# Maaz77/Head-Pose-Estimation-Model

Measured on AMD Instinct MI355X. Metric: images/sec (train+infer) on 96×96 feature maps; yaw/pitch/roll MAE vs ref, higher is better.
Workload: dtype fp32; 1 GPU; Model-96 create_model(num_filters=360, dropout=0, l2=0.1) training, legacy Adam lr 2.8e-4, 96x96 feature maps (configs[3] per GPU: 512 images per rank); global_batch=512, per_gpu_batch=512, positions_per_image=9216, channels=96, parallelism=dp1

## Files before the change

head-pose-estimation-model_amd/csrc/hpe_mlp2.hip:

```cpp
#include <hip/hip_runtime.h>
#include <stdint.h>
#include <stdlib.h>

#include "hpe_common.h"
#include "hpe_dev.h"

#ifdef MLP2_BIG
#define MLP2_NS mlp2_big
#else
#define MLP2_NS mlp2_small
#endif
#define MLP2_BIG_ROWS (1 << 15)
namespace MLP2_NS {

#define MLP2_MAXW 12
#ifndef MLP2_BAR1_SKIP
#define MLP2_BAR1_SKIP 1
#endif
#ifndef MLP2_W88
#define MLP2_W88 2
#endif
#define MLP2_XS 100
#define MLP2_XF (32 * MLP2_XS)
#define MLP2_LAB 128
#define MLP2_RED 32
#define MLP2_FS 104
#define MLP2_TS 40
#define MLP2_A1W (15 * 68 + 64)
#define MLP2_PRE_HALVES (3 * 32 * MLP2_FS + 2 * 3 * 96 * MLP2_TS)

struct E2 {
  int act, drop;
  uint32_t thr;
  float keep;
};

struct TileImg {
  int img0, rem0, P;
  __device__ __forceinline__ int of(int r) const {
    const int t = rem0 + r;
    return img0 + (P >= 32 ? (t >= P ? 1 : 0) : (P == 1 ? t : t / P));
  }
  __device__ __forceinline__ void advance(int dq, int dr) {
    img0 += dq;
    rem0 += dr;
    if (rem0 >= P) { rem0 -= P; ++img0; }
  }
};

__device__ __forceinline__ float e_fwd(const E2& e, uint64_t seed, int64_t img, int ch, float z) {
  float a = act_f(e.act, z);
  if (e.drop >= 0) a = drop_hash(seed, e.drop, (uint64_t)img, ch) >= e.thr ? a / e.keep : 0.f;
  return a;
}

__device__ __forceinline__ float e_bwd(const E2& e, uint64_t seed, int64_t img, int ch, float g, float val) {
  if (e.drop >= 0) {
    if (drop_hash(seed, e.drop, (uint64_t)img, ch) < e.thr) return 0.f;
    g = g / e.keep;
    val = val * e.keep;
  }
  return e.act == ACT_LINEAR ? g : g * act_grad(e.act, val, 0.f);
}
// ... 22 lines not shown
  }
  const int lr = min(lane & 31, last);
  const int limg = ti.of(lr);
  const int lpos = (int)(row0 + lr - (int64_t)limg * P);
  const int lsrc = args.idx ? args.idx[limg] : limg;
  __builtin_amdgcn_s_waitcnt(0x0F70);
  if (labels && wave == 0) {
#pragma unroll
    for (int pc = 0; pc < 2; ++pc) {
      const int slot = pc * 64 + lane;
      const int r = min(slot >> 2, last), j = min(slot & 3, 2);
      const int64_t src = __shfl(lsrc, r, 64);
      glds4(args.ytrue + src * 3 + j, lds_addr(lab + pc * 64));
    }
  }
  for (int r = wave; r < 32; r += NCB) {
    const int rr = min(r, last);
    const int64_t srow = (int64_t)__builtin_amdgcn_readlane(lsrc, rr) * P +
                         __builtin_amdgcn_readlane(lpos, rr);
    if (lane < q) glds16(args.x + srow * Cin + 4 * lane, lds_addr(xs + r * XS));
  }
}

typedef _Float16 h4 __attribute__((ext_vector_type(4)));

__device__ __forceinline__ void split_d4(f32x4 v, h4& ch, h4& cl, h4& h) {
  const f32x4 s = v * SPLIT_C;
  ch = __builtin_convertvector(s, h4);
  cl = __builtin_convertvector(s - __builtin_convertvector(ch, f32x4), h4);
  h = __builtin_convertvector(v, h4);
}
__device__ __forceinline__ constexpr int a1_row(int g) { return 68 * (g ^ ((g >> 1) & 4)); }
template <int KH>
__device__ __forceinline__ void presplit_tile(const float* xs, _Float16* xf, _Float16* xt, int tid, int NT) {
  for (int i = tid; i < 32 * 24; i += NT) {
    const int r = i / 24, rem = i - r * 24, h = rem >= 12 ? 1 : 0, m0 = 4 * (rem - 12 * h);
    const f32x4 v = m0 < KH ? *(const f32x4*)(xs + r * MLP2_XS + KH * h + m0) : f32x4{0.f, 0.f, 0.f, 0.f};
    h4 ch, cl, hh;
    split_d4(v, ch, cl, hh);
    _Float16* d = xf + r * MLP2_FS + 48 * h + m0;
    *(h4*)(d) = ch;
    *(h4*)(d + 32 * MLP2_FS) = cl;
    *(h4*)(d + 64 * MLP2_FS) = hh;
  }
  for (int i = tid; i < 96 * 8; i += NT) {
    const int rg = i / 96, k = i - rg * 96, r = 4 * rg;
    const f32x4 v = {xs[r * MLP2_XS + k], xs[(r + 1) * MLP2_XS + k], xs[(r + 2) * MLP2_XS + k],
                     xs[(r + 3) * MLP2_XS + k]};
    const int p = (r & ~12) | ((r & 4) << 1) | ((r & 8) >> 1);
    h4 ch, cl, hh;
    split_d4(v, ch, cl, hh);
    _Float16* d = xt + k * MLP2_TS + p;
    *(h4*)(d) = ch;
    *(h4*)(d + 96 * MLP2_TS) = cl;
    *(h4*)(d + 192 * MLP2_TS) = hh;
  }
}

template <int KH, int ACT1, bool DROP, int NWM, bool SPLIT>
__global__ void __launch_bounds__(NWM * 64) __attribute__((amdgpu_waves_per_eu(NWM == MLP2_MAXW || ACT1 < 0 ? 1 : MLP2_W88, 8))) mlp2_kernel(Args args) {
  if (!SPLIT && args.guard && __hip_atomic_load(args.guard, __ATOMIC_RELAXED, __HIP_MEMORY_SCOPE_AGENT) != args.epoch) return;
#ifdef MLP2_STAMPS
  const uint64_t rt0 = __builtin_amdgcn_s_memrealtime();
#endif
  extern __shared__ __attribute__((aligned(16))) float lds[];
  constexpr int NKB = (2 * KH + 31) / 32;
  constexpr int T = 32;
  constexpr bool PRE = SPLIT && NWM == MLP2_MAXW;
  constexpr int NXB = PRE ? 1 : 2;
  constexpr bool PAD1 = true;
  constexpr int A1S = MLP2_A1W;
  constexpr int HS = NWM == MLP2_MAXW ? 4 : 3;
  const int* prog = args.prog;
  const int* o = prog + prog[H_OPS_OFF];
  const int mode = prog[H_MODE];
  const bool train = mode == MODE_TRAIN;
  const int Cin = o[O_K], F = o[O_N], NCB = o[O_MODE];
  const int wave = __builtin_amdgcn_readfirstlane(threadIdx.x >> 6);
  const int lane = threadIdx.x & 63, half = lane >> 5, l32 = lane & 31;
  const int NT = blockDim.x;
  const int n = wave * 32 + l32;
  const bool nok = n < F;
  float* xbuf = lds;
  float* lbuf = xbuf + NXB * MLP2_XF;
  float* part = lbuf + 2 * MLP2_LAB;
  float* dz2 = part + NCB * T * 4;
  float* a1s = dz2 + T * 4;
  float* w2t = a1s + NCB * A1S;
  float* b2t = w2t + NCB * 128;
  float* hacc = b2t + 4;
  float* red = hacc + NCB * 64 * HS;
  float* colt = red + MLP2_RED;
  _Float16* xfb = (_Float16*)(colt + NCB * 128);
  _Float16* xtb = xfb + 3 * 32 * MLP2_FS;

  E2 e1 = {o[O_EACT], o[O_EDROP], (uint32_t)o[O_ETHR], __int_as_float(o[O_EKEEP])};
  E2 e2 = {o[O_AUX2], o[O_TBASE], (uint32_t)o[O_TCOUNT], __int_as_float(o[O_F0])};
  const float inv_keep1 = 1.f / e1.keep;
  const float* W1 = args.params + o[O_W];
  const float* W2 = args.params + o[O_AUX0];

  const int64_t nrows = args.nrows;
  const int64_t ntiles = (nrows + T - 1) / T;
  const int P = args.P;
  const bool labels = mode != MODE_FWD;
  const int S = gridDim.x * T, dq = S / P, dr = S - dq * P;
  TileImg ti;
  ti.P = P;
  ti.img0 = (int)(blockIdx.x * T / P);
  ti.rem0 = (int)(blockIdx.x * T - ti.img0 * P);
  if (blockIdx.x < ntiles) stage_tile(args, xbuf, lbuf, (int64_t)blockIdx.x * T, ti, wave, NCB, lane, Cin, labels);
  const int nc = min(n, F - 1);
  const float w2a = W2[nc * 3], w2b = W2[nc * 3 + 1], w2c = W2[nc * 3 + 2];
  const int o_bias = __builtin_amdgcn_readfirstlane(o[O_BIAS]), o_aux1 = __builtin_amdgcn_readfirstlane(o[O_AUX1]);
  const float b1r = args.params[max(o_bias, 0) + nc];
  float w2r[2];
#pragma unroll
  for (int t = 0; t < 2; ++t) {
    const int i = threadIdx.x + t * NT, nn = i >> 2, j = i & 3;
    w2r[t] = W2[min(nn, F - 1) * 3 + min(j, 2)];
  }
  const float b2r = args.params[max(o_aux1, 0) + min((int)threadIdx.x & 3, 2)];

  float wreg[SPLIT ? 1 : KH];
  SplitW wsp[SPLIT ? 6 : 1];
  float inv1 = 1.f, s2 = 1.f;
  if constexpr (SPLIT) {
    f32x8 v[6];
#pragma unroll
    for (int s = 0; s < 6; ++s) {
#pragma unroll
      for (int j = 0; j < 8; ++j) {
        const int k = half * KH + 8 * s + j;
        v[s][j] = 8 * s + j < KH ? W1[(size_t)min(k, Cin - 1) * F + nc] : 0.f;
      }
    }
    __builtin_amdgcn_sched_barrier(0);
    float mx = 0.f;
#pragma unroll
    for (int s = 0; s < 6; ++s) {
#pragma unroll
      for (int j = 0; j < 8; ++j) {
        const int k = half * KH + 8 * s + j;
        v[s][j] = (k < Cin && nok) ? v[s][j] : 0.f;
        mx = fmaxf(mx, fabsf(v[s][j]));
      }
    }
    mx = fmaxf(mx, __shfl_xor(mx, 32, 64));
    const float s1 = pow2_scale(mx, 13);
    inv1 = SPLIT_INV_C / s1;
#pragma unroll
    for (int s = 0; s < 6; ++s) wsp[s] = split_w8(v[s] * s1);
    s2 = pow2_scale(nok ? fmaxf(fmaxf(fabsf(w2a), fabsf(w2b)), fabsf(w2c)) : 0.f, 2);
  } else {
#pragma unroll
    for (int m = 0; m < KH; ++m) {
      const int k = half * KH + m;
      const float wv = W1[(size_t)min(k, Cin - 1) * F + nc];
      wreg[m] = (k < Cin && nok) ? wv : 0.f;
    }
  }
  bool bad = false;
  {
    const float b1 = (nok && o_bias >= 0) ? b1r : 0.f;
    if (half == 0) *(f32x4*)(colt + n * 4) = f32x4{inv1, b1, s2, 0.f};
  }
#pragma unroll
  for (int t = 0; t < 2; ++t) {
    const int i = threadIdx.x + t * NT, nn = i >> 2, j = i & 3;
    if (i < NCB * 128) w2t[i] = (nn < F && j < 3) ? w2r[t] : 0.f;
  }
  if (threadIdx.x < 4) b2t[threadIdx.x] = (threadIdx.x < 3 && o_aux1 >= 0) ? b2r : 0.f;
  for (int i = threadIdx.x; i < NT * HS; i += NT) hacc[i] = 0.f;

  f32x16 dw[NKB];
#pragma unroll
  for (int s = 0; s < NKB; ++s) dw[s] = f32x16{};
  float dw2[3] = {0.f, 0.f, 0.f};
  float db1 = 0.f;

  const int NT3 = (NT / 3) * 3;

  for (int i = threadIdx.x; i < NXB * 32 * 16; i += NT) {
    const int r = i >> 4, c = Cin + (i & 15);
    if (c < 96) xbuf[r * MLP2_XS + c] = 0.f;
  }
  __syncthreads();
  if constexpr (PRE) {
    asm volatile("s_waitcnt vmcnt(0)" ::: "memory");
    bar_lds();
    presplit_tile<KH>(xbuf, xfb, xtb, threadIdx.x, NT);
  }
  int buf = 0;
#ifdef MLP2_STAMPS
  uint32_t ph[9] = {};
  uint64_t tprev = __builtin_amdgcn_s_memtime();
  const uint64_t rt1 = __builtin_amdgcn_s_memrealtime();
#define STAMP(i) do { const uint64_t t_ = __builtin_amdgcn_s_memtime(); ph[i] += (uint32_t)(t_ - tprev); tprev = t_; } while (0)
#else
#define STAMP(i) do {} while (0)
#endif
  for (int tile = blockIdx.x; tile < (int)ntiles; tile += gridDim.x, buf ^= 1, ti.advance(dq, dr)) {
    const int64_t row0 = (int64_t)tile * T;
    const float* xs = xbuf + (PRE ? 0 : buf) * MLP2_XF;
    const float* lab = lbuf + buf * MLP2_LAB;
    if constexpr (!PRE) asm volatile("s_waitcnt vmcnt(0)" ::: "memory");
    STAMP(0);
    if (!(MLP2_BAR1_SKIP && PRE && NCB >= 4 && tile != (int)blockIdx.x)) bar_lds();
    STAMP(1);
    if (tile + gridDim.x < ntiles) {
      TileImg tn = ti;
      tn.advance(dq, dr);
      stage_tile(args, xbuf + (PRE ? 0 : (buf ^ 1)) * MLP2_XF, lbuf + (buf ^ 1) * MLP2_LAB,
                 (int64_t)(tile + gridDim.x) * T, tn, wave, NCB, lane, Cin, labels);
    }

    STAMP(2);
    uint32_t dmask = 0;
    {
      const float* ap = xs + l32 * MLP2_XS + half * KH;
      f32x16 acc = {};
      if constexpr (PRE) {
        const _Float16* fp = xfb + l32 * MLP2_FS + 48 * half;
#pragma unroll
        for (int s = 0; s < 6; ++s) {
          const SplitD xd = {*(const h8*)(fp + 8 * s), *(const h8*)(fp + 32 * MLP2_FS + 8 * s),
                             *(const h8*)(fp + 64 * MLP2_FS + 8 * s)};
          acc = mfma3_dw(xd, wsp[s], acc);
          __builtin_amdgcn_sched_barrier(0);
        }
        bad |= !(fabsf(sum16(acc)) <= 3.0e38f);
        STAMP(3);
      } else if constexpr (SPLIT) {
#pragma unroll
        for (int s = 0; s < 6; ++s) {
          const f32x4 a0 = *(const f32x4*)(ap + 8 * s), a1 = *(const f32x4*)(ap + 8 * s + 4);
          acc = mfma3_dw(split_d8(f32x8{a0.x, a0.y, a0.z, a0.w, a1.x, a1.y, a1.z, a1.w}), wsp[s], acc);
          __builtin_amdgcn_sched_barrier(0);
        }
        bad |= !(fabsf(sum16(acc)) <= 3.0e38f);
      } else {
        f32x4 an = *(const f32x4*)(ap);
#pragma unroll
        for (int m = 0; m < KH; m += 4) {
          const f32x4 a = an;
          if (m + 4 < KH) an = *(const f32x4*)(ap + m + 4);
          acc = __builtin_amdgcn_mfma_f32_32x32x2f32(a.x, wreg[m + 0], acc, 0, 0, 0);
          acc = __builtin_amdgcn_mfma_f32_32x32x2f32(a.y, wreg[m + 1], acc, 0, 0, 0);
          acc = __builtin_amdgcn_mfma_f32_32x32x2f32(a.z, wreg[m + 2], acc, 0, 0, 0);
          acc = __builtin_amdgcn_mfma_f32_32x32x2f32(a.w, wreg[m + 3], acc, 0, 0, 0);
          __builtin_amdgcn_sched_barrier(0);
        }
      }
      if (DROP) {
        if (P >= 32) {
          const bool k0 = drop_hash(args.seed, e1.drop, (uint64_t)(ti.img0 + args.img_off), n) >= e1.thr;
          const bool k1 = drop_hash(args.seed, e1.drop, (uint64_t)(ti.img0 + 1 + args.img_off), n) >= e1.thr;
#pragma unroll
          for (int g = 0; g < 16; ++g) {
            const int r = (g & 3) + 8 * (g >> 2) + 4 * half;
            dmask |= (ti.rem0 + r >= P ? k1 : k0) ? (1u << g) : 0u;
          }
        } else {
#pragma unroll
          for (int g = 0; g < 16; ++g) {
            const int r = (g & 3) + 8 * (g >> 2) + 4 * half;
            dmask |= drop_hash(args.seed, e1.drop, (uint64_t)(ti.of(r) + args.img_off), n) >= e1.thr
                         ? (1u << g) : 0u;
          }
        }
      }
      const f32x4 cs = *(const f32x4*)(colt + n * 4);
#pragma unroll
      for (int g = 0; g < 16; ++g) {
        float z = act1_f<ACT1, SPLIT>(e1.act, SPLIT ? fmaf(acc[g], cs.x, cs.y) : acc[g] + cs.y);
        if (DROP) z = (dmask >> g) & 1u ? z * inv_keep1 : 0.f;
        acc[g] = nok ? z : 0.f;
      }
#pragma unroll
      for (int g = 0; g < 16; ++g) a1s[wave * A1S + (PAD1 ? a1_row(g) : 64 * g) + lane] = acc[g];
      __builtin_amdgcn_fence(__ATOMIC_RELEASE, "wavefront");
      __builtin_amdgcn_wave_barrier();
      __builtin_amdgcn_fence(__ATOMIC_ACQUIRE, "wavefront");
      {
        const int r = l32, hh = (r >> 2) & 1, gr = (r & 3) + 4 * (r >> 3);
        const float* ar = a1s + wave * A1S + (PAD1 ? a1_row(gr) : 64 * gr) + hh * 32 + 16 * half;
        const float* wr = w2t + (wave * 32 + 16 * half) * 4;
        float s0 = 0.f, s1 = 0.f, s2 = 0.f;
#pragma unroll
        for (int i = 0; i < 16; i += 4) {
          const f32x4 av = *(const f32x4*)(ar + i);
#pragma unroll
          for (int e = 0; e < 4; ++e) {
            const f32x4 w = *(const f32x4*)(wr + (i + e) * 4);
            s0 = fmaf(av[e], w.x, s0);
            s1 = fmaf(av[e], w.y, s1);
            s2 = fmaf(av[e], w.z, s2);
          }
        }
        s0 += __shfl_xor(s0, 32, 64);
        s1 += __shfl_xor(s1, 32, 64);
        s2 += __shfl_xor(s2, 32, 64);
        if (half == 0) *(f32x4*)(part + (wave * T + r) * 4) = f32x4{s0, s1, s2, 0.f};
      }
    }
    STAMP(4);
    const bool early = PRE && NCB >= 4;
    if (early) asm volatile("s_waitcnt vmcnt(0)" ::: "memory");
    bar_lds();
    STAMP(5);
    if constexpr (PRE) {
      if (early && wave >= 2 && tile + gridDim.x < ntiles)
        presplit_tile<KH>(xbuf, xfb, xtb + (buf ^ 1) * 3 * 96 * MLP2_TS, threadIdx.x - 128, NT - 128);
    }

    for (int it = threadIdx.x; it < T * 3 && threadIdx.x < NT3; it += NT3) {
      const int r = it / 3, j = it - r * 3;
      const int64_t R = row0 + r;
      float z = b2t[j];
      float pv[MLP2_MAXW];
#pragma unroll
      for (int w = 0; w < MLP2_MAXW; ++w) pv[w] = w < NCB ? part[(w * T + r) * 4 + j] : 0.f;
      float lv = 0.f, ha0 = 0.f, ha1 = 0.f, ha2 = 0.f;
      if (mode != MODE_FWD) {
        lv = lab[r * 4 + j];
        ha0 = hacc[threadIdx.x * HS + 0];
        ha1 = hacc[threadIdx.x * HS + 1];
        ha2 = hacc[threadIdx.x * HS + 2];
      }
#pragma unroll
      for (int w = 0; w < MLP2_MAXW; ++w) z += pv[w];
      const bool d2 = ACT1 < 0 || __builtin_expect(e2.drop >= 0, 0);
      int64_t img = 0;
      bool k2 = true;
      if (d2) {
        img = ti.of(r) + args.img_off;
        if (ACT1 >= 0) k2 = drop_hash(args.seed, e2.drop, (uint64_t)img, j) >= e2.thr;
      }
      const float p = ACT1 >= 0 ? (d2 ? (k2 ? z / e2.keep : 0.f) : z) : e_fwd(e2, args.seed, img, j, z);
      if (mode == MODE_FWD) {
        if (R < nrows) args.y[R * 3 + j] = p;
      } else {
        float g = 0.f;
        if (R < nrows) {
          const float err = p - lv;
          ha0 = fmaf(err, err, ha0);
          ha1 += fabsf(err);
          g = SPLIT ? 2.f * err : 2.f * err * args.inv_count;
        }
        if (train) {
          g = ACT1 >= 0 ? (d2 ? (k2 ? g / e2.keep : 0.f) : g) : e_bwd(e2, args.seed, img, j, g, p);
          dz2[r * 4 + j] = g;
          ha2 += g;
        }
        hacc[threadIdx.x * HS + 0] = ha0;
        hacc[threadIdx.x * HS + 1] = ha1;
        hacc[threadIdx.x * HS + 2] = ha2;
      }
    }
    STAMP(6);
    if constexpr (PRE) {
      asm volatile("s_waitcnt vmcnt(0)" ::: "memory");
      bar_lds();
      STAMP(7);
      if (!early && tile + gridDim.x < ntiles) {
        presplit_tile<KH>(xbuf, xfb, xtb + (buf ^ 1) * 3 * 96 * MLP2_TS, threadIdx.x, NT);
      }
      if (!train) continue;
    } else {
      if (!train) continue;
      bar_lds();
    }

    STAMP(8);
    {
      const f32x4 w2v = *(const f32x4*)(w2t + n * 4);
      const float s2 = colt[n * 4 + 2];
      auto dz_of = [&](int g) {
        const int r = (g & 3) + 8 * (g >> 2) + 4 * half;
        const f32x4 d = *(const f32x4*)(dz2 + r * 4);
        const float a = a1s[wave * A1S + (PAD1 ? a1_row(g) : 64 * g) + lane];
        const float da = d.x * w2v.x + d.y * w2v.y + d.z * w2v.z;
        float gz, av = a;
        if (DROP) {
          gz = (dmask >> g) & 1u ? da * inv_keep1 : 0.f;
          av = a * e1.keep;
        } else {
          gz = da;
        }
        gz = nok ? gz * act1_g<ACT1>(e1.act, av) : 0.f;
        dw2[0] = fmaf(a, d.x, dw2[0]);
        dw2[1] = fmaf(a, d.y, dw2[1]);
        dw2[2] = fmaf(a, d.z, dw2[2]);
        db1 += gz;
        return gz;
      };
      if constexpr (PRE) {
        const _Float16* th = xtb + buf * 3 * 96 * MLP2_TS + l32 * MLP2_TS + 8 * half;
        f32x8 dv0, dv1;
#pragma unroll
        for (int j = 0; j < 8; ++j) dv0[j] = dz_of(j);
        const SplitW d0 = split_w8(dv0 * s2);
        __builtin_amdgcn_sched_barrier(0);
#pragma unroll
        for (int kb = 0; kb < NKB; ++kb) {
          const _Float16* q = th + kb * 32 * MLP2_TS;
          dw[kb] = mfma3_dw(SplitD{*(const h8*)(q), *(const h8*)(q + 96 * MLP2_TS), *(const h8*)(q + 192 * MLP2_TS)}, d0, dw[kb]);
        }
#pragma unroll
        for (int j = 0; j < 8; ++j) dv1[j] = dz_of(8 + j);
        __builtin_amdgcn_sched_barrier(0);
        const SplitW d1 = split_w8(dv1 * s2);
#pragma unroll
        for (int kb = 0; kb < NKB; ++kb) {
          const _Float16* q = th + 16 + kb * 32 * MLP2_TS;
          dw[kb] = mfma3_dw(SplitD{*(const h8*)(q), *(const h8*)(q + 96 * MLP2_TS), *(const h8*)(q + 192 * MLP2_TS)}, d1, dw[kb]);
        }
      } else if constexpr (SPLIT) {
#pragma unroll
        for (int s = 0; s < 2; ++s) {
          f32x8 dv;
#pragma unroll
          for (int j = 0; j < 8; ++j) {
            dv[j] = dz_of(8 * s + j);
            if ((j & 3) == 3) __builtin_amdgcn_sched_barrier(0);
          }
          const SplitW dsp = split_w8(dv * s2);
#pragma unroll
          for (int kb = 0; kb < NKB; ++kb) {
            const float* xp = xs + (4 * half) * MLP2_XS + kb * 32 + l32;
            f32x8 xv;
#pragma unroll
            for (int j = 0; j < 8; ++j) xv[j] = xp[(16 * s + 8 * (j >> 2) + (j & 3)) * MLP2_XS];
            dw[kb] = mfma3_dw(split_d8(xv), dsp, dw[kb]);
            __builtin_amdgcn_sched_barrier(0);
          }
        }
      } else {
        float dz1[16];
#pragma unroll
        for (int g = 0; g < 16; ++g) {
          dz1[g] = dz_of(g);
          if ((g & 3) == 3) __builtin_amdgcn_sched_barrier(0);
        }
#pragma unroll
        for (int kb = 0; kb < NKB; ++kb) {
          const float* xp = xs + (4 * half) * MLP2_XS + kb * 32 + l32;
          f32x16 acc = dw[kb];
          auto xat = [&](int g) { return xp[((g & 3) + 8 * (g >> 2)) * MLP2_XS]; };
          float x0 = xat(0), x1 = xat(1);
#pragma unroll
          for (int g = 0; g < 16; ++g) {
            const float xv = x0;
            x0 = x1;
            if (g + 2 < 16) x1 = xat(g + 2);
            acc = __builtin_amdgcn_mfma_f32_32x32x2f32(xv, dz1[g], acc, 0, 0, 0);
            __builtin_amdgcn_sched_barrier(0);
          }
          dw[kb] = acc;
        }
      }
    }
  }

#ifdef MLP2_STAMPS
  const uint64_t rt2 = __builtin_amdgcn_s_memrealtime();
  uint64_t rtA = 0, rtB = 0;
  if (PRE && blockIdx.x == 0 && lane == 0 && (wave == 0 || wave == 5))
    printf("STAMP w%d bwd+tail %u bar1 %u stage %u fwdmfma %u act+part %u bar2 %u head %u bar3 %u presplit %u\n", wave,
           ph[0], ph[1], ph[2], ph[3], ph[4], ph[5], ph[6], ph[7], ph[8]);
#endif
  if (mode == MODE_FWD) {
    if (SPLIT && bad) __hip_atomic_store(args.guard, args.epoch, __ATOMIC_RELAXED, __HIP_MEMORY_SCOPE_AGENT);
    return;
  }
  const int slab = prog[H_SLAB];
  const int npt = prog[H_NPARAMS_TRAIN];
  float* ws = args.ws + (size_t)blockIdx.x * slab;
  const float sc = SPLIT ? args.inv_count : 1.f;
  const int oW = __builtin_amdgcn_readfirstlane(o[O_W]), oB = __builtin_amdgcn_readfirstlane(o[O_BIAS]);
  const int oA0 = __builtin_amdgcn_readfirstlane(o[O_AUX0]), oA1 = __builtin_amdgcn_readfirstlane(o[O_AUX1]);
  __syncthreads();
  const float s2f = colt[n * 4 + 2];
  if (train) {
    const float scw = SPLIT ? sc * (SPLIT_INV_C / s2f) : sc;
    float chk = 0.f;
#pragma unroll
    for (int kb = 0; kb < NKB; ++kb) {
      if (SPLIT) chk += sum16(dw[kb]);
#pragma unroll
      for (int g = 0; g < 16; ++g) {
        const int k = kb * 32 + (g & 3) + 8 * (g >> 2) + 4 * half;
        if (k < Cin && nok) ws[oW + (size_t)k * F + n] = dw[kb][g] * scw;
      }
    }
    if (SPLIT) bad |= !(fabsf(chk) <= 3.0e38f);
    const float tb = db1 + __shfl_xor(db1, 32, 64);
    float t2[3];
#pragma unroll
    for (int j = 0; j < 3; ++j) t2[j] = dw2[j] + __shfl_xor(dw2[j], 32, 64);
    if (half == 0 && nok) {
      if (oB >= 0) ws[oB + n] = tb * sc;
#pragma unroll
      for (int j = 0; j < 3; ++j) ws[oA0 + n * 3 + j] = t2[j] * sc;
    }
#ifdef MLP2_STAMPS
    rtA = __builtin_amdgcn_s_memrealtime();
#endif
    if (oA1 >= 0) {
      for (int j = wave; j < 3; j += NT >> 6) {
        float s = 0.f;
        for (int i = j + 3 * lane; i < NT3; i += 192) s += hacc[i * HS + 2];
        s = wave_sum(s);
        if (lane == 0) ws[oA1 + j] = s * sc;
      }
    }
#ifdef MLP2_STAMPS
    rtB = __builtin_amdgcn_s_memrealtime();
#endif
    __syncthreads();
  }
#ifdef MLP2_STAMPS
  const uint64_t rtC = __builtin_amdgcn_s_memrealtime();
#endif
  if (SPLIT && bad) __hip_atomic_store(args.guard, args.epoch, __ATOMIC_RELAXED, __HIP_MEMORY_SCOPE_AGENT);
  const float a = wave_sum(hacc[threadIdx.x * HS + 0]), b = wave_sum(hacc[threadIdx.x * HS + 1]);
  if (lane == 0) { red[wave] = a; red[MLP2_MAXW + wave] = b; }
  __syncthreads();
  if (threadIdx.x == 0) {
    float s0 = 0.f, s1 = 0.f;
    const int nw = NT >> 6;
    for (int w = 0; w < nw; ++w) { s0 += red[w]; s1 += red[MLP2_MAXW + w]; }
    ws[npt] = s0;
    ws[npt + 1] = s1;
  }
#ifdef MLP2_STAMPS
  if (PRE && threadIdx.x == 0) {
    const uint64_t rt3 = __builtin_amdgcn_s_memrealtime();
    printf("RT wg %d t0 %llu pro %llu loop %llu flush %llu wstore %llu db2 %llu sync %llu tail %llu\n", (int)blockIdx.x, (unsigned long long)rt0,
           (unsigned long long)(rt1 - rt0), (unsigned long long)(rt2 - rt1), (unsigned long long)(rt3 - rt2),
           (unsigned long long)(rtA - rt2), (unsigned long long)(rtB - rtA), (unsigned long long)(rtC - rtB), (unsigned long long)(rt3 - rtC));
  }
#endif
}

#ifdef MLP2_BIG
#define MLP2R_NU 2
#define MLP2R_LDS_FLOATS (2 * MLP2_XF + 2 * MLP2_LAB + MLP2R_NU * MLP2_A1W + 32 * 4 + MLP2R_NU * 128 + 4)

template <int KH, int ACT1, bool DROP>
// ... 315 lines not shown
    if (half == 0 && nok[u]) {
      if (o_bias >= 0) ws[o_bias + n] = tb * sc;
#pragma unroll
      for (int j = 0; j < 3; ++j) ws[oA0 + n * 3 + j] = t2[j] * sc;
    }
  }
  bad |= !(fabsf(chk) <= 3.0e38f);
#pragma unroll
  for (int j = 0; j < 3; ++j) {
    const float t = wave_sum(db2[j]);
    if (lane == 0 && o_aux1 >= 0) ws[o_aux1 + j] = t * sc;
  }
  if (bad) __hip_atomic_store(args.guard, args.epoch, __ATOMIC_RELAXED, __HIP_MEMORY_SCOPE_AGENT);
  const float ta = wave_sum(sse), tb = wave_sum(sae);
  if (lane == 0) {
    ws[npt] = ta;
    ws[npt + 1] = tb;
  }
}
#endif

typedef void (*mlp2_fn)(Args);

template <int KH, bool DROP, int NWM, bool SPLIT>
static mlp2_fn pick_act(int act, int act2) {
  if (act2 != ACT_LINEAR) return mlp2_kernel<KH, -1, DROP, NWM, SPLIT>;
  if (act == ACT_TANH) return mlp2_kernel<KH, ACT_TANH, DROP, NWM, SPLIT>;
  if (act == ACT_SOFTSIGN) return mlp2_kernel<KH, ACT_SOFTSIGN, DROP, NWM, SPLIT>;
  return mlp2_kernel<KH, -1, DROP, NWM, SPLIT>;
}

template <bool DROP, bool SPLIT>
static mlp2_fn pick_d(int kh, int act, int act2, int ncb) {
  if (ncb <= 4) {
    if (kh == 44) return pick_act<44, DROP, 4, SPLIT>(act, act2);
    if (kh == 48) return pick_act<48, DROP, 4, SPLIT>(act, act2);
  }
  if (kh == 44) return pick_act<44, DROP, MLP2_MAXW, SPLIT>(act, act2);
  if (kh == 48) return pick_act<48, DROP, MLP2_MAXW, SPLIT>(act, act2);
  return nullptr;
}

static mlp2_fn pick(const int* w, bool split = false) {
  const int* o = w + w[H_OPS_OFF];
  const int kh = ((o[O_K] + 7) & ~7) / 2, act = o[O_EACT], act2 = o[O_AUX2];
  if (split)
    return o[O_EDROP] >= 0 ? pick_d<true, true>(kh, act, act2, o[O_MODE]) : pick_d<false, true>(kh, act, act2, o[O_MODE]);
  return o[O_EDROP] >= 0 ? pick_d<true, false>(kh, act, act2, o[O_MODE]) : pick_d<false, false>(kh, act, act2, o[O_MODE]);
}

static void geom(const int* w, int& kh, int& rbw, int& ncb, int& lds_bytes, int& act, int& drop) {
  const int* o = w + w[H_OPS_OFF];
  act = o[O_EACT];
  drop = o[O_EDROP];
  const int cin = o[O_K];
  const int cp = (cin + 7) & ~7;
  kh = cp / 2;
  rbw = o[O_FLAGS];
  ncb = o[O_MODE];
  const int T = 32;
  const int rest = 2 * MLP2_LAB + ncb * T * 4 + T * 4 + ncb * MLP2_A1W + ncb * 128 + 4 + ncb * 64 * (ncb > 4 ? 4 : 3) + MLP2_RED + ncb * 128;
  lds_bytes = (2 * MLP2_XF + rest) * 4;
  const int pre = (MLP2_XF + rest) * 4 + MLP2_PRE_HALVES * 2;
  if (ncb > 4 && pre > lds_bytes) lds_bytes = pre;
}

static int lds_split(const int* w) {
  int kh, rbw, ncb, lds, act, drop;
  geom(w, kh, rbw, ncb, lds, act, drop);
  return lds;
}

static int launch_k(mlp2_fn k, int nw, int lds, const Args& a, int grid, hipStream_t s) {
  hipFuncSetAttribute((const void*)k, hipFuncAttributeMaxDynamicSharedMemorySize, lds);
  hipLaunchKernelGGL(k, dim3(grid), dim3(nw * 64), lds, s, a);
  return hipGetLastError() == hipSuccess ? 0 : 2;
}

static bool split_only() {
  const char* e = getenv("HPE_SPLIT_ONLY");
  return e && e[0] == '1';
}

#ifdef MLP2_BIG
// ... 11 lines not shown
  const int kh = ((o[O_K] + 7) & ~7) / 2;
  if (kh == 44 && o[O_K] == 88) return pick_r_act<44>(o[O_EACT], o[O_EDROP] >= 0);
  if (kh == 48) return pick_r_act<48>(o[O_EACT], o[O_EDROP] >= 0);
  return nullptr;
}
#else
static mlp2_fn pick_r(const int*) { return nullptr; }
#define MLP2R_LDS_FLOATS 0
#endif

static int launch_pair(const int* w, const Args& a, int grid, hipStream_t s) {
  int kh, rbw, ncb, lds, act, drop;
  geom(w, kh, rbw, ncb, lds, act, drop);
  if (hpe_exact_fp32() || !a.guard) {
    Args e = a;
    e.guard = nullptr;
    const int tv = hpe_tev_begin(s);
    const int rc = launch_k(pick(w), ncb, lds, e, grid, s);
    hpe_tev_end(s, tv);
    return rc;
  }
  const mlp2_fn kr = pick_r(w);
  const int tv = hpe_tev_begin(s);
  const int rc = kr ? launch_k(kr, 1, MLP2R_LDS_FLOATS * 4, a, grid, s) : launch_k(pick(w, true), ncb, lds_split(w), a, grid, s);
  hpe_tev_end(s, tv);
  if (rc) return rc;
  if (split_only()) return 0;
  if (a.x_bound > 0.f && a.x_bound < SPLIT_DATA_RANGE) return 0;
  return launch_k(pick(w), ncb, lds, a, grid, s);
}

static int per_cu_of(mlp2_fn k, int ncb, int lds) {
  hipFuncAttributes attr;
  int per_cu = 1;
  if (hipFuncGetAttributes(&attr, (const void*)k) == hipSuccess) {
    const int vg = ((attr.numRegs + 7) / 8) * 8;
    const int waves_simd = vg > 0 ? (512 / vg > 8 ? 8 : 512 / vg) : 8;
    per_cu = (4 * waves_simd) / ncb;
  }
  const int by_lds = (160 * 1024) / lds;
  if (per_cu > by_lds) per_cu = by_lds;
  return per_cu < 1 ? 1 : per_cu;
}

static int cap_per_cu(const int* w) {
  int kh, rbw, ncb, lds, act, drop;
  geom(w, kh, rbw, ncb, lds, act, drop);
  const int a = per_cu_of(pick(w), ncb, lds), b = per_cu_of(pick(w, true), ncb, lds_split(w));
  const mlp2_fn kr = pick_r(w);
  const int c = kr ? per_cu_of(kr, 1, MLP2R_LDS_FLOATS * 4) : b;
  return a < b ? (a < c ? a : c) : (b < c ? b : c);
}
}

#ifdef MLP2_BIG
int mlp2_launch_big(const int* w, const Args& a, int grid, hipStream_t s) {
  return MLP2_NS::launch_pair(w, a, grid, s);
}
int mlp2_per_cu_big(const int* w) { return MLP2_NS::cap_per_cu(w); }
#else
using namespace MLP2_NS;
int mlp2_launch_big(const int* w, const Args& a, int grid, hipStream_t s);
int mlp2_per_cu_big(const int* w);

int mlp2_supported(const int* w) {
  int kh, rbw, ncb, lds, act, drop;
  geom(w, kh, rbw, ncb, lds, act, drop);
  const int* o = w + w[H_OPS_OFF];
  return pick(w) != nullptr && rbw == 1 && ncb >= 1 && ncb <= MLP2_MAXW &&
         o[O_AUX3] == 3 && (o[O_K] & 3) == 0 && o[O_K] <= 96 && lds <= 160 * 1024;
}

int mlp2_grid_cap(const int* w, int n_cu) {
  const int a = MLP2_NS::cap_per_cu(w), b = mlp2_per_cu_big(w);
// ... 9 lines not shown
```

Before: 177,400 images/sec.

## Add contiguous-row staging variant for pre-split MLP2 kernel with cheaper overflow checks

Adds a CONTIG instantiation of the pre-split MLP2 kernel, used when there is no index array and P>=32. It stages input rows by pointer stride instead of per-row readlane address math, and loads labels by image offset. The overflow guard moves from a per-tile MFMA accumulator sum to range checks on the inputs and weights. Other changes: fp16 fragment loads are software-pipelined across MFMA steps, the partial sums are padded to the max wave count, and the s2 scaling is folded into w2 so two multiplies drop from the backward pass. These cut staging overhead and per-tile checks, at the cost of more template instantiations and subtle numeric-guard semantics.

```diff
diff --git a/head-pose-estimation-model_amd/csrc/hpe_mlp2.hip b/head-pose-estimation-model_amd/csrc/hpe_mlp2.hip
--- a/head-pose-estimation-model_amd/csrc/hpe_mlp2.hip
+++ b/head-pose-estimation-model_amd/csrc/hpe_mlp2.hip
@@ -37,8 +37,10 @@
 
 struct TileImg {
   int img0, rem0, P;
+  template <bool P32 = false>
   __device__ __forceinline__ int of(int r) const {
     const int t = rem0 + r;
+    if (P32) return img0 + (t >= P ? 1 : 0);
     return img0 + (P >= 32 ? (t >= P ? 1 : 0) : (P == 1 ? t : t / P));
   }
   __device__ __forceinline__ void advance(int dq, int dr) {
@@ -107,6 +109,32 @@
   }
 }
 
+__device__ __forceinline__ int lane_now() {
+  int l;
+  asm volatile("v_mbcnt_lo_u32_b32 %0, -1, 0\n\tv_mbcnt_hi_u32_b32 %0, -1, %0" : "=v"(l));
+  return l;
+}
+
+__device__ __forceinline__ void stage_contig(const Args& args, float* xs, float* lab, const float* tp,
+                                             int64_t row0, const TileImg& ti, int wave, int NCB, int Cin,
+                                             bool labels) {
+  const int lane = lane_now();
+  const int64_t rem = args.nrows - 1 - row0;
+  const int last = rem < 31 ? (int)rem : 31;
+  if (labels && wave == 0) {
+    const float* yp = args.ytrue + (int64_t)ti.img0 * 3;
+#pragma unroll
+    for (int pc = 0; pc < 2; ++pc) {
+      const int slot = pc * 64 + lane;
+      const int r = min(slot >> 2, last), j = min(slot & 3, 2);
+      glds4(yp + (ti.rem0 + r >= ti.P ? 3 + j : j), lds_addr(lab + pc * 64));
+    }
+  }
+  const int q = Cin >> 2;
+  for (int r = wave; r < 32; r += NCB)
+    if (lane < q) glds16(tp + min(r, last) * Cin + 4 * lane, lds_addr(xs + r * MLP2_XS));
+}
+
 typedef _Float16 h4 __attribute__((ext_vector_type(4)));
 
 __device__ __forceinline__ void split_d4(f32x4 v, h4& ch, h4& cl, h4& h) {
@@ -116,11 +144,15 @@
   h = __builtin_convertvector(v, h4);
 }
 __device__ __forceinline__ constexpr int a1_row(int g) { return 68 * (g ^ ((g >> 1) & 4)); }
+#define MLP2_X_LIMIT (65520.f / SPLIT_C)
 template <int KH>
-__device__ __forceinline__ void presplit_tile(const float* xs, _Float16* xf, _Float16* xt, int tid, int NT) {
+__device__ __forceinline__ bool presplit_tile(const float* xs, _Float16* xf, _Float16* xt, int tid, int NT) {
+  bool out = false;
   for (int i = tid; i < 32 * 24; i += NT) {
     const int r = i / 24, rem = i - r * 24, h = rem >= 12 ? 1 : 0, m0 = 4 * (rem - 12 * h);
     const f32x4 v = m0 < KH ? *(const f32x4*)(xs + r * MLP2_XS + KH * h + m0) : f32x4{0.f, 0.f, 0.f, 0.f};
+    out |= !(fabsf(v.x) < MLP2_X_LIMIT) | !(fabsf(v.y) < MLP2_X_LIMIT) | !(fabsf(v.z) < MLP2_X_LIMIT) |
+           !(fabsf(v.w) < MLP2_X_LIMIT);
     h4 ch, cl, hh;
     split_d4(v, ch, cl, hh);
     _Float16* d = xf + r * MLP2_FS + 48 * h + m0;
@@ -140,10 +172,12 @@
     *(h4*)(d + 96 * MLP2_TS) = cl;
     *(h4*)(d + 192 * MLP2_TS) = hh;
   }
-}
-
-template <int KH, int ACT1, bool DROP, int NWM, bool SPLIT>
+  return out;
+}
+
+template <int KH, int ACT1, bool DROP, int NWM, bool SPLIT, bool CONTIG = false>
 __global__ void __launch_bounds__(NWM * 64) __attribute__((amdgpu_waves_per_eu(NWM == MLP2_MAXW || ACT1 < 0 ? 1 : MLP2_W88, 8))) mlp2_kernel(Args args) {
+  static_assert(!CONTIG || (SPLIT && NWM == MLP2_MAXW), "CONTIG is an instantiation of the pre-split kernel");
   if (!SPLIT && args.guard && __hip_atomic_load(args.guard, __ATOMIC_RELAXED, __HIP_MEMORY_SCOPE_AGENT) != args.epoch) return;
 #ifdef MLP2_STAMPS
   const uint64_t rt0 = __builtin_amdgcn_s_memrealtime();
@@ -153,6 +187,7 @@
   constexpr int T = 32;
   constexpr bool PRE = SPLIT && NWM == MLP2_MAXW;
   constexpr int NXB = PRE ? 1 : 2;
+  constexpr bool LEAN = PRE && ACT1 >= 0;
   constexpr bool PAD1 = true;
   constexpr int A1S = MLP2_A1W;
   constexpr int HS = NWM == MLP2_MAXW ? 4 : 3;
@@ -166,10 +201,11 @@
   const int NT = blockDim.x;
   const int n = wave * 32 + l32;
   const bool nok = n < F;
+  const int NPR = NWM == MLP2_MAXW ? MLP2_MAXW : NCB;
   float* xbuf = lds;
   float* lbuf = xbuf + NXB * MLP2_XF;
   float* part = lbuf + 2 * MLP2_LAB;
-  float* dz2 = part + NCB * T * 4;
+  float* dz2 = part + NPR * T * 4;
   float* a1s = dz2 + T * 4;
   float* w2t = a1s + NCB * A1S;
   float* b2t = w2t + NCB * 128;
@@ -194,7 +230,13 @@
   ti.P = P;
   ti.img0 = (int)(blockIdx.x * T / P);
   ti.rem0 = (int)(blockIdx.x * T - ti.img0 * P);
-  if (blockIdx.x < ntiles) stage_tile(args, xbuf, lbuf, (int64_t)blockIdx.x * T, ti, wave, NCB, lane, Cin, labels);
+  const float* xnext = CONTIG ? args.x + (int64_t)blockIdx.x * T * Cin : nullptr;
+  const int64_t xstep = CONTIG ? (int64_t)gridDim.x * T * Cin : 0;
+  if (blockIdx.x < ntiles) {
+    if constexpr (CONTIG) stage_contig(args, xbuf, lbuf, xnext, (int64_t)blockIdx.x * T, ti, wave, NCB, Cin, labels);
+    else stage_tile(args, xbuf, lbuf, (int64_t)blockIdx.x * T, ti, wave, NCB, lane, Cin, labels);
+  }
+  xnext += xstep;
   const int nc = min(n, F - 1);
   const float w2a = W2[nc * 3], w2b = W2[nc * 3 + 1], w2c = W2[nc * 3 + 2];
   const int o_bias = __builtin_amdgcn_readfirstlane(o[O_BIAS]), o_aux1 = __builtin_amdgcn_readfirstlane(o[O_AUX1]);
@@ -210,6 +252,7 @@
   float wreg[SPLIT ? 1 : KH];
   SplitW wsp[SPLIT ? 6 : 1];
   float inv1 = 1.f, s2 = 1.f;
+  bool wbad = false;
   if constexpr (SPLIT) {
     f32x8 v[6];
 #pragma unroll
@@ -235,7 +278,14 @@
     const float s1 = pow2_scale(mx, 13);
     inv1 = SPLIT_INV_C / s1;
 #pragma unroll
-    for (int s = 0; s < 6; ++s) wsp[s] = split_w8(v[s] * s1);
+    for (int s = 0; s < 6; ++s) {
+      const f32x8 vs = v[s] * s1;
+      wsp[s] = split_w8(vs);
+      if (PRE) {
+#pragma unroll
+        for (int j = 0; j < 8; ++j) wbad |= !(fabsf(vs[j]) < 65520.f);
+      }
+    }
     s2 = pow2_scale(nok ? fmaxf(fmaxf(fabsf(w2a), fabsf(w2b)), fabsf(w2c)) : 0.f, 2);
   } else {
 #pragma unroll
@@ -245,7 +295,7 @@
       wreg[m] = (k < Cin && nok) ? wv : 0.f;
     }
   }
-  bool bad = false;
+  bool bad = PRE && wbad && blockIdx.x < ntiles;
   {
     const float b1 = (nok && o_bias >= 0) ? b1r : 0.f;
     if (half == 0) *(f32x4*)(colt + n * 4) = f32x4{inv1, b1, s2, 0.f};
@@ -270,11 +320,13 @@
     const int r = i >> 4, c = Cin + (i & 15);
     if (c < 96) xbuf[r * MLP2_XS + c] = 0.f;
   }
+  for (int i = NCB * T * 4 + threadIdx.x; i < NPR * T * 4; i += NT) part[i] = 0.f;
   __syncthreads();
   if constexpr (PRE) {
     asm volatile("s_waitcnt vmcnt(0)" ::: "memory");
     bar_lds();
-    presplit_tile<KH>(xbuf, xfb, xtb, threadIdx.x, NT);
+    const bool xbad = presplit_tile<KH>(xbuf, xfb, xtb, threadIdx.x, NT);
+    bad |= xbad && blockIdx.x < ntiles;
   }
   int buf = 0;
 #ifdef MLP2_STAMPS
@@ -286,6 +338,9 @@
 #define STAMP(i) do {} while (0)
 #endif
   for (int tile = blockIdx.x; tile < (int)ntiles; tile += gridDim.x, buf ^= 1, ti.advance(dq, dr)) {
+    const int tlane = PRE ? lane_now() : lane, thalf = tlane >> 5, tl32 = tlane & 31;
+    const int tcol = wave * 32 + tl32;
+    const bool tok = tcol < F;
     const int64_t row0 = (int64_t)tile * T;
     const float* xs = xbuf + (PRE ? 0 : buf) * MLP2_XF;
     const float* lab = lbuf + buf * MLP2_LAB;
@@ -296,25 +351,36 @@
     if (tile + gridDim.x < ntiles) {
       TileImg tn = ti;
       tn.advance(dq, dr);
-      stage_tile(args, xbuf + (PRE ? 0 : (buf ^ 1)) * MLP2_XF, lbuf + (buf ^ 1) * MLP2_LAB,
-                 (int64_t)(tile + gridDim.x) * T, tn, wave, NCB, lane, Cin, labels);
+      if constexpr (CONTIG) {
+        stage_contig(args, xbuf, lbuf + (buf ^ 1) * MLP2_LAB, xnext, (int64_t)(tile + gridDim.x) * T, tn,
+                     wave, NCB, Cin, labels);
+        xnext += xstep;
+      } else {
+        stage_tile(args, xbuf + (PRE ? 0 : (buf ^ 1)) * MLP2_XF, lbuf + (buf ^ 1) * MLP2_LAB,
+                   (int64_t)(tile + gridDim.x) * T, tn, wave, NCB, tlane, Cin, labels);
+      }
     }
 
     STAMP(2);
     uint32_t dmask = 0;
     {
-      const float* ap = xs + l32 * MLP2_XS + half * KH;
+      const float* ap = xs + tl32 * MLP2_XS + thalf * KH;
       f32x16 acc = {};
       if constexpr (PRE) {
-        const _Float16* fp = xfb + l32 * MLP2_FS + 48 * half;
+        const _Float16* fp = xfb + tl32 * MLP2_FS + 48 * thalf;
+        auto frag = [&](int s) {
+          return SplitD{*(const h8*)(fp + 8 * s), *(const h8*)(fp + 32 * MLP2_FS + 8 * s),
+                        *(const h8*)(fp + 64 * MLP2_FS + 8 * s)};
+        };
+        SplitD xd = frag(0);
 #pragma unroll
         for (int s = 0; s < 6; ++s) {
-          const SplitD xd = {*(const h8*)(fp + 8 * s), *(const h8*)(fp + 32 * MLP2_FS + 8 * s),
-                             *(const h8*)(fp + 64 * MLP2_FS + 8 * s)};
+          SplitD xn = xd;
+          if (s + 1 < 6) xn = frag(s + 1);
+          __builtin_amdgcn_sched_barrier(0);
           acc = mfma3_dw(xd, wsp[s], acc);
-          __builtin_amdgcn_sched_barrier(0);
-        }
-        bad |= !(fabsf(sum16(acc)) <= 3.0e38f);
+          xd = xn;
+        }
         STAMP(3);
       } else if constexpr (SPLIT) {
 #pragma unroll
@@ -338,39 +404,39 @@
         }
       }
       if (DROP) {
-        if (P >= 32) {
-          const bool k0 = drop_hash(args.seed, e1.drop, (uint64_t)(ti.img0 + args.img_off), n) >= e1.thr;
-          const bool k1 = drop_hash(args.seed, e1.drop, (uint64_t)(ti.img0 + 1 + args.img_off), n) >= e1.thr;
+        if (CONTIG || P >= 32) {
+          const bool k0 = drop_hash(args.seed, e1.drop, (uint64_t)(ti.img0 + args.img_off), tcol) >= e1.thr;
+          const bool k1 = drop_hash(args.seed, e1.drop, (uint64_t)(ti.img0 + 1 + args.img_off), tcol) >= e1.thr;
 #pragma unroll
           for (int g = 0; g < 16; ++g) {
-            const int r = (g & 3) + 8 * (g >> 2) + 4 * half;
+            const int r = (g & 3) + 8 * (g >> 2) + 4 * thalf;
             dmask |= (ti.rem0 + r >= P ? k1 : k0) ? (1u << g) : 0u;
           }
         } else {
 #pragma unroll
           for (int g = 0; g < 16; ++g) {
-            const int r = (g & 3) + 8 * (g >> 2) + 4 * half;
-            dmask |= drop_hash(args.seed, e1.drop, (uint64_t)(ti.of(r) + args.img_off), n) >= e1.thr
+            const int r = (g & 3) + 8 * (g >> 2) + 4 * thalf;
+            dmask |= drop_hash(args.seed, e1.drop, (uint64_t)(ti.of(r) + args.img_off), tcol) >= e1.thr
                          ? (1u << g) : 0u;
           }
         }
       }
-      const f32x4 cs = *(const f32x4*)(colt + n * 4);
+      const f32x4 cs = *(const f32x4*)(colt + tcol * 4);
 #pragma unroll
       for (int g = 0; g < 16; ++g) {
         float z = act1_f<ACT1, SPLIT>(e1.act, SPLIT ? fmaf(acc[g], cs.x, cs.y) : acc[g] + cs.y);
         if (DROP) z = (dmask >> g) & 1u ? z * inv_keep1 : 0.f;
-        acc[g] = nok ? z : 0.f;
-      }
-#pragma unroll
-      for (int g = 0; g < 16; ++g) a1s[wave * A1S + (PAD1 ? a1_row(g) : 64 * g) + lane] = acc[g];
+        acc[g] = LEAN || tok ? z : 0.f;
+      }
+#pragma unroll
+      for (int g = 0; g < 16; ++g) a1s[wave * A1S + (PAD1 ? a1_row(g) : 64 * g) + tlane] = acc[g];
       __builtin_amdgcn_fence(__ATOMIC_RELEASE, "wavefront");
       __builtin_amdgcn_wave_barrier();
       __builtin_amdgcn_fence(__ATOMIC_ACQUIRE, "wavefront");
       {
-        const int r = l32, hh = (r >> 2) & 1, gr = (r & 3) + 4 * (r >> 3);
-        const float* ar = a1s + wave * A1S + (PAD1 ? a1_row(gr) : 64 * gr) + hh * 32 + 16 * half;
-        const float* wr = w2t + (wave * 32 + 16 * half) * 4;
+        const int r = tl32, hh = (r >> 2) & 1, gr = (r & 3) + 4 * (r >> 3);
+        const float* ar = a1s + wave * A1S + (PAD1 ? a1_row(gr) : 64 * gr) + hh * 32 + 16 * thalf;
+        const float* wr = w2t + (wave * 32 + 16 * thalf) * 4;
         float s0 = 0.f, s1 = 0.f, s2 = 0.f;
 #pragma unroll
         for (int i = 0; i < 16; i += 4) {
@@ -386,7 +452,7 @@
         s0 += __shfl_xor(s0, 32, 64);
         s1 += __shfl_xor(s1, 32, 64);
         s2 += __shfl_xor(s2, 32, 64);
-        if (half == 0) *(f32x4*)(part + (wave * T + r) * 4) = f32x4{s0, s1, s2, 0.f};
+        if (thalf == 0) *(f32x4*)(part + (wave * T + r) * 4) = f32x4{s0, s1, s2, 0.f};
       }
     }
     STAMP(4);
@@ -396,16 +462,16 @@
     STAMP(5);
     if constexpr (PRE) {
       if (early && wave >= 2 && tile + gridDim.x < ntiles)
-        presplit_tile<KH>(xbuf, xfb, xtb + (buf ^ 1) * 3 * 96 * MLP2_TS, threadIdx.x - 128, NT - 128);
-    }
-
-    for (int it = threadIdx.x; it < T * 3 && threadIdx.x < NT3; it += NT3) {
+        bad |= presplit_tile<KH>(xbuf, xfb, xtb + (buf ^ 1) * 3 * 96 * MLP2_TS, threadIdx.x - 128, NT - 128);
+    }
+
+    auto head_item = [&](int it) {
       const int r = it / 3, j = it - r * 3;
       const int64_t R = row0 + r;
       float z = b2t[j];
       float pv[MLP2_MAXW];
 #pragma unroll
-      for (int w = 0; w < MLP2_MAXW; ++w) pv[w] = w < NCB ? part[(w * T + r) * 4 + j] : 0.f;
+      for (int w = 0; w < MLP2_MAXW; ++w) pv[w] = NWM == MLP2_MAXW || w < NCB ? part[(w * T + r) * 4 + j] : 0.f;
       float lv = 0.f, ha0 = 0.f, ha1 = 0.f, ha2 = 0.f;
       if (mode != MODE_FWD) {
         lv = lab[r * 4 + j];
@@ -419,7 +485,7 @@
       int64_t img = 0;
       bool k2 = true;
       if (d2) {
-        img = ti.of(r) + args.img_off;
+        img = ti.of<CONTIG>(r) + args.img_off;
         if (ACT1 >= 0) k2 = drop_hash(args.seed, e2.drop, (uint64_t)img, j) >= e2.thr;
       }
       const float p = ACT1 >= 0 ? (d2 ? (k2 ? z / e2.keep : 0.f) : z) : e_fwd(e2, args.seed, img, j, z);
@@ -442,6 +508,11 @@
         hacc[threadIdx.x * HS + 1] = ha1;
         hacc[threadIdx.x * HS + 2] = ha2;
       }
+    };
+    if constexpr (NWM == MLP2_MAXW) {
+      if (threadIdx.x < T * 3) head_item(threadIdx.x);
+    } else {
+      for (int it = threadIdx.x; it < T * 3 && threadIdx.x < NT3; it += NT3) head_item(it);
     }
     STAMP(6);
     if constexpr (PRE) {
@@ -449,7 +520,7 @@
       bar_lds();
       STAMP(7);
       if (!early && tile + gridDim.x < ntiles) {
-        presplit_tile<KH>(xbuf, xfb, xtb + (buf ^ 1) * 3 * 96 * MLP2_TS, threadIdx.x, NT);
+        bad |= presplit_tile<KH>(xbuf, xfb, xtb + (buf ^ 1) * 3 * 96 * MLP2_TS, threadIdx.x, NT);
       }
       if (!train) continue;
     } else {
@@ -459,13 +530,15 @@
 
     STAMP(8);
     {
-      const f32x4 w2v = *(const f32x4*)(w2t + n * 4);
-      const float s2 = colt[n * 4 + 2];
+      const f32x4 w2r = *(const f32x4*)(w2t + tcol * 4);
+      const float s2 = colt[tcol * 4 + 2];
+      const f32x4 w2v = PRE ? f32x4{w2r.x * s2, w2r.y * s2, w2r.z * s2, 0.f} : w2r;
       auto dz_of = [&](int g) {
-        const int r = (g & 3) + 8 * (g >> 2) + 4 * half;
+        const int r = (g & 3) + 8 * (g >> 2) + 4 * thalf;
         const f32x4 d = *(const f32x4*)(dz2 + r * 4);
-        const float a = a1s[wave * A1S + (PAD1 ? a1_row(g) : 64 * g) + lane];
-        const float da = d.x * w2v.x + d.y * w2v.y + d.z * w2v.z;
+        const float a = a1s[wave * A1S + (PAD1 ? a1_row(g) : 64 * g) + tlane];
+        const float da = PRE ? fmaf(d.z, w2v.z, fmaf(d.x, w2v.x, d.y * w2v.y))
+                             : d.x * w2v.x + d.y * w2v.y + d.z * w2v.z;
         float gz, av = a;
         if (DROP) {
           gz = (dmask >> g) & 1u ? da * inv_keep1 : 0.f;
@@ -473,19 +546,22 @@
         } else {
           gz = da;
         }
-        gz = nok ? gz * act1_g<ACT1>(e1.act, av) : 0.f;
+        {
+#pragma clang fp contract(off)
+          gz = LEAN || tok ? gz * act1_g<ACT1>(e1.act, av) : 0.f;
+          db1 += gz;
+        }
         dw2[0] = fmaf(a, d.x, dw2[0]);
         dw2[1] = fmaf(a, d.y, dw2[1]);
         dw2[2] = fmaf(a, d.z, dw2[2]);
-        db1 += gz;
         return gz;
       };
       if constexpr (PRE) {
-        const _Float16* th = xtb + buf * 3 * 96 * MLP2_TS + l32 * MLP2_TS + 8 * half;
+        const _Float16* th = xtb + buf * 3 * 96 * MLP2_TS + tl32 * MLP2_TS + 8 * thalf;
         f32x8 dv0, dv1;
 #pragma unroll
         for (int j = 0; j < 8; ++j) dv0[j] = dz_of(j);
-        const SplitW d0 = split_w8(dv0 * s2);
+        const SplitW d0 = split_w8(dv0);
         __builtin_amdgcn_sched_barrier(0);
 #pragma unroll
         for (int kb = 0; kb < NKB; ++kb) {
@@ -495,7 +571,7 @@
 #pragma unroll
         for (int j = 0; j < 8; ++j) dv1[j] = dz_of(8 + j);
         __builtin_amdgcn_sched_barrier(0);
-        const SplitW d1 = split_w8(dv1 * s2);
+        const SplitW d1 = split_w8(dv1);
 #pragma unroll
         for (int kb = 0; kb < NKB; ++kb) {
           const _Float16* q = th + 16 + kb * 32 * MLP2_TS;
@@ -513,7 +589,7 @@
           const SplitW dsp = split_w8(dv * s2);
 #pragma unroll
           for (int kb = 0; kb < NKB; ++kb) {
-            const float* xp = xs + (4 * half) * MLP2_XS + kb * 32 + l32;
+            const float* xp = xs + (4 * thalf) * MLP2_XS + kb * 32 + tl32;
             f32x8 xv;
 #pragma unroll
             for (int j = 0; j < 8; ++j) xv[j] = xp[(16 * s + 8 * (j >> 2) + (j & 3)) * MLP2_XS];
@@ -530,7 +606,7 @@
         }
 #pragma unroll
         for (int kb = 0; kb < NKB; ++kb) {
-          const float* xp = xs + (4 * half) * MLP2_XS + kb * 32 + l32;
+          const float* xp = xs + (4 * thalf) * MLP2_XS + kb * 32 + tl32;
           f32x16 acc = dw[kb];
           auto xat = [&](int g) { return xp[((g & 3) + 8 * (g >> 2)) * MLP2_XS]; };
           float x0 = xat(0), x1 = xat(1);
@@ -555,6 +631,9 @@
     printf("STAMP w%d bwd+tail %u bar1 %u stage %u fwdmfma %u act+part %u bar2 %u head %u bar3 %u presplit %u\n", wave,
            ph[0], ph[1], ph[2], ph[3], ph[4], ph[5], ph[6], ph[7], ph[8]);
 #endif
+  const int flane = PRE ? lane_now() : lane, fhalf = flane >> 5;
+  const int fcol = wave * 32 + (flane & 31);
+  const bool fok = fcol < F;
   if (mode == MODE_FWD) {
     if (SPLIT && bad) __hip_atomic_store(args.guard, args.epoch, __ATOMIC_RELAXED, __HIP_MEMORY_SCOPE_AGENT);
     return;
@@ -566,7 +645,7 @@
   const int oW = __builtin_amdgcn_readfirstlane(o[O_W]), oB = __builtin_amdgcn_readfirstlane(o[O_BIAS]);
   const int oA0 = __builtin_amdgcn_readfirstlane(o[O_AUX0]), oA1 = __builtin_amdgcn_readfirstlane(o[O_AUX1]);
   __syncthreads();
-  const float s2f = colt[n * 4 + 2];
+  const float s2f = colt[fcol * 4 + 2];
   if (train) {
     const float scw = SPLIT ? sc * (SPLIT_INV_C / s2f) : sc;
     float chk = 0.f;
@@ -575,19 +654,19 @@
       if (SPLIT) chk += sum16(dw[kb]);
 #pragma unroll
       for (int g = 0; g < 16; ++g) {
-        const int k = kb * 32 + (g & 3) + 8 * (g >> 2) + 4 * half;
-        if (k < Cin && nok) ws[oW + (size_t)k * F + n] = dw[kb][g] * scw;
-      }
-    }
-    if (SPLIT) bad |= !(fabsf(chk) <= 3.0e38f);
-    const float tb = db1 + __shfl_xor(db1, 32, 64);
+        const int k = kb * 32 + (g & 3) + 8 * (g >> 2) + 4 * fhalf;
+        if (k < Cin && fok) ws[oW + (size_t)k * F + fcol] = dw[kb][g] * scw;
+      }
+    }
+    if (SPLIT) bad |= (!LEAN || fok) && !(fabsf(chk) <= 3.0e38f);
+    const float tb = (db1 + __shfl_xor(db1, 32, 64)) * (PRE ? 1.f / s2f : 1.f);
     float t2[3];
 #pragma unroll
     for (int j = 0; j < 3; ++j) t2[j] = dw2[j] + __shfl_xor(dw2[j], 32, 64);
-    if (half == 0 && nok) {
-      if (oB >= 0) ws[oB + n] = tb * sc;
-#pragma unroll
-      for (int j = 0; j < 3; ++j) ws[oA0 + n * 3 + j] = t2[j] * sc;
+    if (fhalf == 0 && fok) {
+      if (oB >= 0) ws[oB + fcol] = tb * sc;
+#pragma unroll
+      for (int j = 0; j < 3; ++j) ws[oA0 + fcol * 3 + j] = t2[j] * sc;
     }
 #ifdef MLP2_STAMPS
     rtA = __builtin_amdgcn_s_memrealtime();
@@ -595,9 +674,9 @@
     if (oA1 >= 0) {
       for (int j = wave; j < 3; j += NT >> 6) {
         float s = 0.f;
-        for (int i = j + 3 * lane; i < NT3; i += 192) s += hacc[i * HS + 2];
+        for (int i = j + 3 * flane; i < NT3; i += 192) s += hacc[i * HS + 2];
         s = wave_sum(s);
-        if (lane == 0) ws[oA1 + j] = s * sc;
+        if (flane == 0) ws[oA1 + j] = s * sc;
       }
     }
 #ifdef MLP2_STAMPS
@@ -610,7 +689,7 @@
 #endif
   if (SPLIT && bad) __hip_atomic_store(args.guard, args.epoch, __ATOMIC_RELAXED, __HIP_MEMORY_SCOPE_AGENT);
   const float a = wave_sum(hacc[threadIdx.x * HS + 0]), b = wave_sum(hacc[threadIdx.x * HS + 1]);
-  if (lane == 0) { red[wave] = a; red[MLP2_MAXW + wave] = b; }
+  if (flane == 0) { red[wave] = a; red[MLP2_MAXW + wave] = b; }
   __syncthreads();
   if (threadIdx.x == 0) {
     float s0 = 0.f, s1 = 0.f;
@@ -972,31 +1051,35 @@
 
 typedef void (*mlp2_fn)(Args);
 
-template <int KH, bool DROP, int NWM, bool SPLIT>
+template <int KH, bool DROP, int NWM, bool SPLIT, bool CONTIG = false>
 static mlp2_fn pick_act(int act, int act2) {
-  if (act2 != ACT_LINEAR) return mlp2_kernel<KH, -1, DROP, NWM, SPLIT>;
-  if (act == ACT_TANH) return mlp2_kernel<KH, ACT_TANH, DROP, NWM, SPLIT>;
-  if (act == ACT_SOFTSIGN) return mlp2_kernel<KH, ACT_SOFTSIGN, DROP, NWM, SPLIT>;
-  return mlp2_kernel<KH, -1, DROP, NWM, SPLIT>;
+  if (act2 != ACT_LINEAR) return mlp2_kernel<KH, -1, DROP, NWM, SPLIT, CONTIG>;
+  if (act == ACT_TANH) return mlp2_kernel<KH, ACT_TANH, DROP, NWM, SPLIT, CONTIG>;
+  if (act == ACT_SOFTSIGN) return mlp2_kernel<KH, ACT_SOFTSIGN, DROP, NWM, SPLIT, CONTIG>;
+  return mlp2_kernel<KH, -1, DROP, NWM, SPLIT, CONTIG>;
 }
 
 template <bool DROP, bool SPLIT>
-static mlp2_fn pick_d(int kh, int act, int act2, int ncb) {
+static mlp2_fn pick_d(int kh, int act, int act2, int ncb, bool contig) {
   if (ncb <= 4) {
     if (kh == 44) return pick_act<44, DROP, 4, SPLIT>(act, act2);
     if (kh == 48) return pick_act<48, DROP, 4, SPLIT>(act, act2);
   }
+  if constexpr (SPLIT) {
+    if (contig && kh == 44) return pick_act<44, DROP, MLP2_MAXW, SPLIT, true>(act, act2);
+    if (contig && kh == 48) return pick_act<48, DROP, MLP2_MAXW, SPLIT, true>(act, act2);
+  }
   if (kh == 44) return pick_act<44, DROP, MLP2_MAXW, SPLIT>(act, act2);
   if (kh == 48) return pick_act<48, DROP, MLP2_MAXW, SPLIT>(act, act2);
   return nullptr;
 }
 
-static mlp2_fn pick(const int* w, bool split = false) {
+static mlp2_fn pick(const int* w, bool split = false, bool contig = false) {
   const int* o = w + w[H_OPS_OFF];
   const int kh = ((o[O_K] + 7) & ~7) / 2, act = o[O_EACT], act2 = o[O_AUX2];
   if (split)
-    return o[O_EDROP] >= 0 ? pick_d<true, true>(kh, act, act2, o[O_MODE]) : pick_d<false, true>(kh, act, act2, o[O_MODE]);
-  return o[O_EDROP] >= 0 ? pick_d<true, false>(kh, act, act2, o[O_MODE]) : pick_d<false, false>(kh, act, act2, o[O_MODE]);
+    return o[O_EDROP] >= 0 ? pick_d<true, true>(kh, act, act2, o[O_MODE], contig) : pick_d<false, true>(kh, act, act2, o[O_MODE], contig);
+  return o[O_EDROP] >= 0 ? pick_d<true, false>(kh, act, act2, o[O_MODE], false) : pick_d<false, false>(kh, act, act2, o[O_MODE], false);
 }
 
 static void geom(const int* w, int& kh, int& rbw, int& ncb, int& lds_bytes, int& act, int& drop) {
@@ -1009,7 +1092,8 @@
   rbw = o[O_FLAGS];
   ncb = o[O_MODE];
   const int T = 32;
-  const int rest = 2 * MLP2_LAB + ncb * T * 4 + T * 4 + ncb * MLP2_A1W + ncb * 128 + 4 + ncb * 64 * (ncb > 4 ? 4 : 3) + MLP2_RED + ncb * 128;
+  const int npr = ncb > 4 ? MLP2_MAXW : ncb;
+  const int rest = 2 * MLP2_LAB + npr * T * 4 + T * 4 + ncb * MLP2_A1W + ncb * 128 + 4 + ncb * 64 * (ncb > 4 ? 4 : 3) + MLP2_RED + ncb * 128;
   lds_bytes = (2 * MLP2_XF + rest) * 4;
   const int pre = (MLP2_XF + rest) * 4 + MLP2_PRE_HALVES * 2;
   if (ncb > 4 && pre > lds_bytes) lds_bytes = pre;
@@ -1067,7 +1151,8 @@
   }
   const mlp2_fn kr = pick_r(w);
   const int tv = hpe_tev_begin(s);
-  const int rc = kr ? launch_k(kr, 1, MLP2R_LDS_FLOATS * 4, a, grid, s) : launch_k(pick(w, true), ncb, lds_split(w), a, grid, s);
+  const bool contig = a.idx == nullptr && a.P >= 32;
+  const int rc = kr ? launch_k(kr, 1, MLP2R_LDS_FLOATS * 4, a, grid, s) : launch_k(pick(w, true, contig), ncb, lds_split(w), a, grid, s);
   hpe_tev_end(s, tv);
   if (rc) return rc;
   if (split_only()) return 0;
@@ -1091,10 +1176,16 @@
 static int cap_per_cu(const int* w) {
   int kh, rbw, ncb, lds, act, drop;
   geom(w, kh, rbw, ncb, lds, act, drop);
-  const int a = per_cu_of(pick(w), ncb, lds), b = per_cu_of(pick(w, true), ncb, lds_split(w));
+  int cap = per_cu_of(pick(w), ncb, lds);
+  const int b = per_cu_of(pick(w, true), ncb, lds_split(w)), bc = per_cu_of(pick(w, true, true), ncb, lds_split(w));
+  cap = b < cap ? b : cap;
+  cap = bc < cap ? bc : cap;
   const mlp2_fn kr = pick_r(w);
-  const int c = kr ? per_cu_of(kr, 1, MLP2R_LDS_FLOATS * 4) : b;
-  return a < b ? (a < c ? a : c) : (b < c ? b : c);
+  if (kr) {
+    const int c = per_cu_of(kr, 1, MLP2R_LDS_FLOATS * 4);
+    cap = c < cap ? c : cap;
+  }
+  return cap;
 }
 }
 
```

Result: faster. 186,100 images/sec (median of 6 runs) (+4.9%).
